# mjq11302010044/TPGSR

Measured on AMD Instinct MI355X. Metric: training img/s (16x64->32x128, bs=48/GPU), TPGSR-TSRN full train step, higher is better.
Workload: dtype bf16x2; 1 GPU; C3: TPGSR-TSRN = TSRN_TL (STN+mask) + CRNN teacher/student text prior, stu_iter 1, full train step (teacher fwd, student fwd+bwd, distill loss, prior dropout, SR fwd+bwd, ImageLoss(gradient), clip 0.25, Adam); tpg=crnn, batch_per_gpu=48, global_batch=48, parallelism=dp1, launch=recorded plans, plain launches: main + weight-gradient + teacher streams

## Files before the change

include/tpgsr_hip.h:

```cpp
#ifndef TPGSR_HIP_H
#define TPGSR_HIP_H

#ifdef __cplusplus
extern "C" {
#endif

#define TPGSR_ACT_NONE 0
#define TPGSR_ACT_RELU 1
#define TPGSR_ACT_MISH 2
#define TPGSR_ACT_TANH 3
#define TPGSR_ACT_PRELU 4

const char* tpgsr_last_error(void);
int tpgsr_version(void);
int tpgsr_sizeof(int which);

typedef struct {
  const float* in;
  const float* in2;
  const float* in_scale;
  const float* in_shift;
  const float* wt;
  const float* bias;
  float* out;
  float* bn_partial;
  int N, H, W, Cin;
// ... 137 lines not shown
  float* dwih0;
  float* dwih1;
  float* dbih0;
  float* dbih1;
  int Cin, U, G, blk0;
} tpgsr_compose_bwd_desc;
int tpgsr_compose_bwd_blocks(int Cin, int U, int G);
int tpgsr_compose_bwd_program(const tpgsr_compose_bwd_desc* descs_dev, int ndesc, int total_blocks, void* stream);
int tpgsr_pack_blocks(int kind, int Cout, int Cin, int KH, int KW, long long numel);
int tpgsr_pack_program(const tpgsr_pack_desc* descs_dev, int ndesc, int total_blocks, void* stream);
typedef struct tpgsr_split_desc {
  const float* src;
  void* dst;
  int K, N, ld, kp, blk0;
  int cin;
} tpgsr_split_desc;
int tpgsr_split_bf_blocks(int K, int N);
int tpgsr_split_bf_program(const tpgsr_split_desc* descs_dev, int ndesc, int total_blocks, void* stream);
int tpgsr_bicubic_resize(const float* in_nchw, int N, int Ctot, int C, int H, int W, int OH, int OW, float scale, float shift,
                         float* out_nhwc, void* stream);
int tpgsr_bicubic_upsample(const float* in_nchw, int N, int Ctot, int C, int H, int W, int scale, float* out_nchw, void* stream);
int tpgsr_aster_attention(const float* xproj, const float* sproj, const float* wv, const float* bv, const float* x, int N, int T, int A,
                          int D, float* alpha, float* context, void* stream);
int tpgsr_embed_concat(const int* ids, const float* emb, int V, int E, const float* ctx, int D, int N, float* out, void* stream);
int tpgsr_gru_cell(const float* gi, const float* gh, const float* h, int N, int Hd, float* hnew, void* stream);
int tpgsr_softmax_max(const float* logits, int N, int C, int* ids, float* score, int ld, int col, int* ids_next, void* stream);
int tpgsr_aster_attention_rows(const float* xproj, const float* sproj, const float* wv, const float* bv, const float* x, int R,
                               int rows_per_seq, int T, int A, int D, float* alpha, float* context, void* stream);
int tpgsr_beam_step(const float* logits, float* seq, int N, int B, int C, int eos, float* score_t, int* sym_t, int* pred_t, void* stream);
int tpgsr_gather_rows(const float* src, const int* idx, int R, int W, float* dst, void* stream);
// ... 247 lines not shown
```

tpgsr_amd/csrc/conv_loader.h:

```cpp
#pragma once
#include "common.h"

#define BM 64
#define BN 64
#define KC 32
#define ALD (BM + 1)

__device__ __forceinline__ int xcd_remap(int L, int total) {
  int q = total >> 3, r = total & 7;
  int xcd = L & 7, j = L >> 3;
  return (xcd < r ? xcd * (q + 1) : r * (q + 1) + (xcd - r) * q) + j;
}

struct PixelPos {
  int n, oh, ow;
  bool valid;
};

__device__ __forceinline__ PixelPos decode_pixel(const tpgsr_conv_args& a, int m, int M) {
  PixelPos p;
  p.valid = m < M;
  int mm = p.valid ? m : 0;
  int ohw = a.OH * a.OW;
  p.n = mm / ohw;
// ... 108 lines not shown
  s.dr = dk - dq * a.Cin;
  s.dqh = dq / a.KW;
  s.dqw = dq - s.dqh * a.KW;
  return s;
}
__device__ __forceinline__ void kpos_advance(const tpgsr_conv_args& a, KPos& k, const KStep& s) {
  k.c += s.dr;
  const bool cc = k.c >= a.Cin;
  k.c -= cc ? a.Cin : 0;
  k.kw += s.dqw + (cc ? 1 : 0);
  const bool cw = k.kw >= a.KW;
  k.kw -= cw ? a.KW : 0;
  k.kh += s.dqh + (cw ? 1 : 0);
}

template <int LD>
__device__ __forceinline__ ARaw load_a_raw(const tpgsr_conv_args& a, __amdgpu_buffer_rsrc_t rin, __amdgpu_buffer_rsrc_t rin2,
                                           const PixelPos& p, const KPos& kp) {
  ARaw r;
  const int kh = kp.kh, kw = kp.kw, c = kp.c;
  int ih = p.oh + kh - a.pad_h, iw = p.ow * stride_w(a) + kw - a.pad_w;
  r.ok = p.valid && kh < a.KH && c < a.Cin && (unsigned)ih < (unsigned)a.H && (unsigned)iw < (unsigned)a.W;
  int Wr = a.W;
  if (a.in_dil_w > 1) {
    r.ok = r.ok && (iw % a.in_dil_w) == 0;
    iw /= a.in_dil_w;
    Wr = real_w(a);
  }
  const unsigned pix = (unsigned)((p.n * a.H + ih) * Wr + iw);
  if ((LD & 16) && c >= a.cin_a) {
    r.v = buf_load4(rin2, r.ok ? (((unsigned)p.n * (unsigned)Wr + (unsigned)iw) * (unsigned)a.in_b_ld + (unsigned)(c - a.cin_a)) * 4u : OOB_OFF);
    r.v2 = make_float4(0.f, 0.f, 0.f, 0.f);
    r.raw = true;
    return r;
  }
  r.raw = false;
  if (!(LD & 8)) {
    r.v = buf_load4(rin, r.ok ? (pix * (unsigned)a.in_ld + (unsigned)(a.in_coff + c)) * 4u : OOB_OFF);
  } else {
    unsigned C4 = (unsigned)a.Cin >> 2, cs = (unsigned)c >> 2, W2 = 2u * (unsigned)a.W;
    unsigned b = r.ok ? ((((unsigned)p.n * 2u * a.H + 2u * ih) * W2 + 2u * iw) * C4 + cs) * 4u : OOB_OFF;
    r.v.x = buf_load1(rin, b);
    r.v.y = buf_load1(rin, r.ok ? b + C4 * 4u : OOB_OFF);
    r.v.z = buf_load1(rin, r.ok ? b + W2 * C4 * 4u : OOB_OFF);
    r.v.w = buf_load1(rin, r.ok ? b + (W2 * C4 + C4) * 4u : OOB_OFF);
  }
  if (LD & 4) r.v2 = buf_load4(rin2, r.ok ? (pix * (unsigned)a.in2_ld + (unsigned)c) * 4u : OOB_OFF);
  return r;
}

template <int LD>
__device__ __forceinline__ float4 finish_a(const tpgsr_conv_args& a, const ARaw& r, const float4& s, const float4& t,
                                           const float4& s2 = make_float4(1.f, 1.f, 1.f, 1.f)) {
// ... 35 lines not shown
```

tpgsr_amd/csrc/conv_mfma.hip:

```cpp
#include "common.h"
#include <mutex>

#ifndef TPGSR_FRAG_PRELOAD
#define TPGSR_FRAG_PRELOAD 0
#endif
#include <utility>
#include <vector>
#include "conv_loader.h"
#include "conv_launch.h"

template <int LD, int SPLIT>
__global__ __launch_bounds__(256 * SPLIT) void conv_fwd_kernel(tpgsr_conv_args a, int M, int K, int vecB) {
  constexpr bool VEC_A = LD >= 0;
  __shared__ float As_[SPLIT][KC][ALD];
  __shared__ float Bs_[SPLIT][KC][BN];
  const int grp = SPLIT > 1 ? (int)(threadIdx.x >> 8) : 0;
  float (*As)[ALD] = As_[grp];
  float (*Bs)[BN] = Bs_[grp];
  const int tid = threadIdx.x & 255;
  const int lane = tid & 63, wave = tid >> 6;
  const int wm = wave & 1, wn = wave >> 1;
  const int nbn = (a.Cout + BN - 1) / BN;
  const int tile = xcd_remap(blockIdx.x, gridDim.x);
  const int mblk = tile / nbn;
// ... 324 lines not shown
  long long M = (long long)a->N * a->OH * a->OW;
  int K = a->KH * a->KW * a->Cin;
  TPGSR_CHECK_ARG(M < (1ll << 31), "tpgsr_conv_fwd: M too large");
  hipStream_t st = (hipStream_t)stream;
  if (a->bnb_y) {
    TPGSR_CHECK_ARG(!a->out_ps && !a->bias && a->out_act == TPGSR_ACT_NONE,
                    "tpgsr_conv_fwd: bnb_y goes with a plain dense data-gradient store (no bias, no output activation, no pixel shuffle)");
    TPGSR_CHECK_ARG(a->bnb_act == TPGSR_ACT_NONE || a->bnb_act == TPGSR_ACT_RELU || a->bnb_act == TPGSR_ACT_MISH, "tpgsr_conv_fwd: bnb_act %d", a->bnb_act);
    TPGSR_CHECK_ARG((a->bnb_scale == nullptr) == (a->bnb_shift == nullptr), "tpgsr_conv_fwd: bnb_scale / bnb_shift must come together");
    if (a->bn_partial)
      TPGSR_CHECK_ARG(a->bnb_mean && a->bnb_rstd && (a->bnb_act == TPGSR_ACT_NONE || a->bnb_scale),
                      "tpgsr_conv_fwd: BatchNorm-backward sums need bnb_mean, bnb_rstd (and bnb_scale / bnb_shift under an activation)");
    else
      TPGSR_CHECK_ARG(a->bnb_store_dz, "tpgsr_conv_fwd: bnb_y without bn_partial and without bnb_store_dz does nothing");
  }
  const bool xbf = xbf_eligible(a);
  if (xbf) {
    TPGSR_CHECK_ARG(a->terms >= 1 && a->terms <= 3, "tpgsr_conv_fwd: terms must be 0, 1, 2 or 3");
    TPGSR_CHECK_ARG(a->kp >= K && (a->kp & 31) == 0 && ((uintptr_t)a->wt_bf & 15) == 0, "tpgsr_conv_fwd: bad split operand (kp %d, K %d)", a->kp, K);
    TPGSR_CHECK_ARG(a->wt_bf_cin == 0 || (a->wt_bf_cin == a->Cin && (a->Cin & 31) == 0),
                    "tpgsr_conv_fwd: weights were split in channel-block order for Cin %d, the convolution has Cin %d", a->wt_bf_cin, a->Cin);
  } else {
    TPGSR_CHECK_ARG(a->bn_row_tiles <= 1, "tpgsr_conv_fwd: bn_row_tiles %d needs the whole-CU halo kernel (split-bf16 path)", a->bn_row_tiles);
    TPGSR_CHECK_ARG(!a->bnb_y, "tpgsr_conv_fwd: the BatchNorm-backward epilogue (bnb_y) exists in the split-bf16 kernels only (terms > 0, wt_bf, Cin %% 4 == 0)");
  }
  const tpgsr_conv_route_t r = conv_fwd_route(a, M);
  if (xbf && a->sk_splits <= 1 && r.kernel != TPGSR_CONV_XBF_HALO3) {
    TPGSR_CHECK_ARG(!(r.ld & 32), "tpgsr_conv_fwd: a scaled residual operand (in2_scale) exists in the whole-CU halo kernel's loader only, which does not "
                    "take this launch (ask tpgsr_conv_in2_scale_ok first)");
    TPGSR_CHECK_ARG(a->bn_row_tiles <= 1, "tpgsr_conv_fwd: bn_row_tiles %d is the whole-CU halo kernel's, which does not take this launch "
                    "(ask tpgsr_conv_bn_row_tiles first)", a->bn_row_tiles);
  }
  dim3 grid(cdiv(M, BM) * cdiv(a->Cout, BN));
  switch (r.kernel) {
    case TPGSR_CONV_XBF_SPLITK:
    case TPGSR_CONV_XBF_TILE: return conv_fwd_xbf_launch(a, M, K, r, st);
// ... 741 lines not shown
```

tpgsr_amd/csrc/conv_xbf.hip:

```cpp
#include "conv_loader.h"
#include <type_traits>
#include <utility>
#include <vector>
#include <mutex>

#include "conv_xbf_common.h"

__device__ __forceinline__ int xa_off(int row, int slot) { return row * 64 + ((slot ^ ((row >> 2) & 3)) << 4); }

template <int LD, int T, int WMB, int WNB, int SK = 0>
__global__ __launch_bounds__(256, (WMB * WNB == 1 ? 3 : WMB * WNB == 2 ? 2 : 1)) void conv_fwd_xbf_kernel(tpgsr_conv_args a, int M, int K) {
  constexpr int BMT = 64 * WMB, BNT = 64 * WNB;
  constexpr int A_PLANE = BMT * 64;
  constexpr int BUF = T * A_PLANE;
  constexpr int NQ = BMT / 32;
  constexpr bool TWO = (T == 3) && (WMB * WNB <= 2);
  constexpr int EPI = (4 * 64 * WNB + 4 * 1024) * 4;
  __shared__ __attribute__((aligned(16))) unsigned char xsm[2 * BUF > EPI ? 2 * BUF : EPI];
  const int tid = threadIdx.x;
  const int lane = tid & 63, wave = tid >> 6;
  const int wm = wave & 1, wn = wave >> 1;
  const int nbn = (a.Cout + BNT - 1) / BNT;
  const int ntile = SK ? (int)gridDim.x / a.sk_splits : (int)gridDim.x;
  const int skz = SK ? (int)blockIdx.x / ntile : 0;
// ... 33 lines not shown
  ARaw qa[NQ];
  float4 qs = make_float4(1.f, 1.f, 1.f, 1.f), qt = make_float4(0.f, 0.f, 0.f, 0.f);
  const bool kperm = a.wt_bf_cin > 0;
  KPos kp_ = kperm ? KPos{0, 0, aq * 4} : kpos_init(a, aq);
  if (SK && c0 > 0) {
    if (kperm) {
      const int taps = a.KH * a.KW, cb = c0 / taps, tp = c0 - cb * taps;
      kp_ = KPos{tp / a.KW, tp - (tp / a.KW) * a.KW, cb * 32 + aq * 4};
    } else {
      kpos_advance(a, kp_, c0 * KC);
    }
  }
  const KStep kstep = kstep_init(a, KC);
  auto load_chunk = [&]() {
#pragma unroll
    for (int i = 0; i < NQ; ++i) qa[i] = load_a_raw<LD>(a, rs_in, rs_in2, px[i], kp_);
    if (LD & 1) {
      qs = *reinterpret_cast<const float4*>(a.in_scale + ((kp_.kh < a.KH && kp_.c < a.Cin) ? kp_.c : 0));
      qt = *reinterpret_cast<const float4*>(a.in_shift + ((kp_.kh < a.KH && kp_.c < a.Cin) ? kp_.c : 0));
    }
    if (kperm) {
      const bool cw = ++kp_.kw >= a.KW;
      kp_.kw = cw ? 0 : kp_.kw;
      kp_.kh += cw ? 1 : 0;
      const bool chh = kp_.kh >= a.KH;
      kp_.kh = chh ? 0 : kp_.kh;
      kp_.c += chh ? 32 : 0;
    } else {
      kpos_advance(a, kp_, kstep);
    }
  };
// ... 240 lines not shown
      }
    };
    constexpr bool DB = !(LD & 4);
    ARaw hr[DB ? 2 : 1][NE];
    float4 qs[2], qt[2];
    qs[0] = qs[1] = make_float4(1.f, 1.f, 1.f, 1.f);
    qt[0] = qt[1] = make_float4(0.f, 0.f, 0.f, 0.f);
    auto load_item = [&](auto set_tag, const int cc) __attribute__((always_inline)) {
      constexpr int S = decltype(set_tag)::value;
      const int c = cc * 32 + aq * 4;
#pragma unroll
      for (int i = 0; i < NE; ++i) {
        const bool ok = hpix[i] >= 0;
        hr[S][i].ok = ok;
        hr[S][i].raw = hpix[i] > -2;
        if (LD & 8) {
          const unsigned C4 = (unsigned)a.Cin >> 2, W2 = 2u * (unsigned)a.W;
          const unsigned b = ok ? ((2u * (unsigned)hpix[i] * W2 + 2u * (unsigned)hcol[i]) * C4 + ((unsigned)c >> 2)) * 4u : OOB_OFF;
          hr[S][i].v.x = buf_load1(rs_in, b);
          hr[S][i].v.y = buf_load1(rs_in, ok ? b + C4 * 4u : OOB_OFF);
          hr[S][i].v.z = buf_load1(rs_in, ok ? b + W2 * C4 * 4u : OOB_OFF);
          hr[S][i].v.w = buf_load1(rs_in, ok ? b + (W2 * C4 + C4) * 4u : OOB_OFF);
        } else {
          hr[S][i].v = buf_load4(rs_in, ok ? ((unsigned)hpix[i] * (unsigned)a.in_ld + (unsigned)(a.in_coff + c)) * 4u : OOB_OFF);
        }
        if (LD & 4) hr[S][i].v2 = buf_load4(rs_in2, ok ? ((unsigned)hpix[i] * (unsigned)a.in2_ld + (unsigned)c) * 4u : OOB_OFF);
      }
      if (LD & 1) {
        qs[S] = *reinterpret_cast<const float4*>(a.in_scale + c);
        qt[S] = *reinterpret_cast<const float4*>(a.in_shift + c);
      }
// ... 683 lines not shown
  const int lane = threadIdx.x & 63;
  const long long b = (long long)blockIdx.x * 4 + (threadIdx.x >> 6);
  if (b >= (long long)MB16 * NB32) return;
  const int mb = (int)(b / NB32), nb = (int)(b - (long long)mb * NB32);
  const int n = nb * 32 + (lane & 31), p0 = mb * 16 + (lane >> 5) * 8;
  __bf16 h[8][T];
#pragma unroll
  for (int j = 0; j < 8; ++j) {
    const int m = p0 + j;
    float v = 0.f;
    if (m < M && n < Cout) {
      if (!dy_ps) {
        v = dy[(size_t)m * dy_ld + dy_coff + n];
      } else {
        const int ohw = OH * OW, nn = m / ohw, rem = m - nn * ohw, oh = rem / OW, ow = rem - oh * OW;
        v = dy[((size_t)(nn * 2 * OH + 2 * oh + ((n >> 1) & 1)) * (2 * OW) + 2 * ow + (n & 1)) * (Cout >> 2) + (n >> 2)];
      }
    }
    split_bf<T>(v, h[j]);
  }
  const size_t plane = (size_t)MB16 * NB32 * 512;
#pragma unroll
  for (int t = 0; t < T; ++t) {
    bf16x8 v;
#pragma unroll
    for (int j = 0; j < 8; ++j) v[j] = h[j][t];
    *reinterpret_cast<bf16x8*>(out + t * plane + ((size_t)b * 64 + lane) * 8) = v;
  }
}

struct FastDiv {
// ... 234 lines not shown
          }
        }
      }
    };
    if (!(dbg & 1)) {
      step(I0{}, 0, t * 4 + 0);
      step(I1{}, 1, t * 4 + 1);
      step(I0{}, 2, t * 4 + 2);
      step(I1{}, 3, t * 4 + 3);
    }
  }

  const int n = n0 + wn * 32 + (lane & 31);
  float* dst = w.part + (size_t)z * K * a.Cout;
  if (n < a.Cout) {
#pragma unroll
    for (int i = 0; i < 3; ++i)
      if (i < ntap) {
#pragma unroll
        for (int r = 0; r < 16; ++r) {
          const int k = (tap0 + i) * a.Cin + cc * 32 + (r & 3) + 8 * (r >> 2) + 4 * (lane >> 5);
          dst[(size_t)k * a.Cout + n] = acc[i][r];
        }
      }
    if (want_db && lane < 32) w.dbpart[(size_t)z * a.Cout + n] = accdb[0];
  }
}

extern "C" int tpgsr_wgrad_halo_plan(const tpgsr_conv_args* a, int* zsplits, long long* dy_bf_bytes) {
  if (!a) return 0;
  int cus = 256, dev = 0;
  if (hipGetDevice(&dev) == hipSuccess) (void)hipDeviceGetAttribute(&cus, hipDeviceAttributeMultiprocessorCount, dev);
  if (cus < 1) cus = 256;
  return wgrad_halo_plan(a, cus, zsplits, dy_bf_bytes);
}

int conv_wgrad_halo_launch(const tpgsr_wgrad_args* w, long long M, const tpgsr_wgrad_route_t& r, hipStream_t st) {
  const tpgsr_conv_args* a = &w->c;
  const int T = a->terms, ld = r.ld, Lcap = r.lcap;
  const size_t lds = r.lds_bytes;
// ... 53 lines not shown
  __syncthreads();
  const tpgsr_split_desc d = descs[s_d];
  const int b = (int)blockIdx.x - d.blk0;
  const int nkb = d.kp / 64 + ((d.kp & 63) ? 1 : 0);
  const int kb = b % nkb, nbk = b / nkb;
  const int k0 = kb * 64, n0 = nbk * 64;
  {
    const int n = threadIdx.x & 63, kr = threadIdx.x >> 6;
#pragma unroll
    for (int i = 0; i < 16; ++i) {
      int k = k0 + kr * 16 + i;
      if (d.cin > 0 && k < d.K) {
        const int taps = d.K / d.cin, cc = k / (taps * 32), rem = k - cc * taps * 32;
        k = (rem >> 5) * d.cin + cc * 32 + (rem & 31);
      }
      tile[kr * 16 + i][n] = (k < d.K && n0 + n < d.N) ? d.src[(size_t)k * d.ld + n0 + n] : 0.f;
    }
  }
  __syncthreads();
  const int NB32 = (d.N + 31) >> 5, KB16 = d.kp >> 4;
  unsigned short* dst = reinterpret_cast<unsigned short*>(d.dst);
  const size_t plane = (size_t)NB32 * KB16 * 512;
  for (int i = 0; i < 2; ++i) {
    const int p = threadIdx.x + 256 * i;
    const int n = p & 63, kg = p >> 6;
    const int k = k0 + kg * 8, nn = n0 + n;
    if (k >= d.kp || nn >= NB32 * 32) continue;
    __bf16 h[8][3];
#pragma unroll
    for (int j = 0; j < 8; ++j) split_bf<3>(tile[kg * 8 + j][n], h[j]);
    const size_t off = ((((size_t)(nn >> 5) * KB16 + (k >> 4)) * 64) + ((k >> 3) & 1) * 32 + (nn & 31)) * 8;
// ... 60 lines not shown
```

tpgsr_amd/csrc/conv_xbf_common.h:

```cpp
#pragma once
#include "conv_loader.h"
#include "conv_launch.h"

typedef __bf16 bf16x8 __attribute__((ext_vector_type(8)));
typedef __bf16 bf16x4 __attribute__((ext_vector_type(4)));
typedef short s16x4 __attribute__((ext_vector_type(4)));
typedef __attribute__((address_space(3))) s16x4* lds_s16x4_ptr;

#define XW_ROW 192
#define XW_PLANE (32 * XW_ROW)

template <int T>
__device__ __forceinline__ void split_bf(float x, __bf16 (&h)[T]) {
  h[0] = (__bf16)x;
  if (T > 1) {
    float r = x - (float)h[0];
    h[1] = (__bf16)r;
    if (T > 2) h[2] = (__bf16)(r - (float)h[1]);
  }
}
template <int T>
__device__ __forceinline__ void split4(const float4& v, uint2 (&out)[T]) {
  __bf16 a[T], b[T], c[T], d[T];
  split_bf<T>(v.x, a);
// ... 22 lines not shown
    acc = __builtin_amdgcn_mfma_f32_32x32x16_bf16(a[1], b[0], acc, 0, 0, 0);
  }
  return __builtin_amdgcn_mfma_f32_32x32x16_bf16(a[0], b[0], acc, 0, 0, 0);
}

#ifndef XBF_NT_STORE
#define XBF_NT_STORE 0
#endif
__device__ __forceinline__ float xbf_bnb_elem(float raw, float y, float sc, float sh, float mu, float rs, int act, float& s, float& ss) {
  const float dz = act ? raw * act_grad(__builtin_fmaf(y, sc, sh), act) : raw;
  s += dz;
  ss = __builtin_fmaf(dz * (y - mu), rs, ss);
  return dz;
}

template <int WMB, int WNB>
__device__ __forceinline__ void xbf_store_tile(const tpgsr_conv_args& a, floatx16 (&acc)[WMB][WNB], int M, int m0, int n0, int wm,
                                               int wn, int lane, float* red) {
  constexpr int BNT = 64 * WNB;
  const int ohw = a.OH * a.OW;
#pragma unroll
  for (int j = 0; j < WNB; ++j) {
    const int cloc = wn * 32 * WNB + 32 * j + (lane & 31);
    const int n = n0 + cloc;
    const bool nvalid = n < a.Cout;
    const float bias = (a.bias && nvalid) ? a.bias[n] : 0.f;
    float s = 0.f, ss = 0.f;
    const bool bnb = a.bnb_y != nullptr;
    float b_mu = 0.f, b_rs = 0.f, b_sc = 1.f, b_sh = 0.f;
    if (bnb && nvalid) {
      if (a.bn_partial) {
        b_mu = a.bnb_mean[n];
        b_rs = a.bnb_rstd[n];
// ... 112 lines not shown
__device__ __forceinline__ void xbf_bn_flush(const tpgsr_conv_args& a, int M, int n0, int mblk, int tid, const float* red) {
  constexpr int BNT = 64 * WNB;
  for (int e = tid; e < BNT * WMB; e += 256) {
    const int blk = e / BNT, c = e - blk * BNT;
    const long long rb64 = (long long)mblk * WMB + blk;
    if (n0 + c < a.Cout && rb64 * 64 < M) {
      float* dst = a.bn_partial + (size_t)rb64 * 2 * a.Cout;
      float v0, v1;
      if (WMB == 1) {
        v0 = red[0 * BNT + c] + red[2 * BNT + c];
        v1 = red[1 * BNT + c] + red[3 * BNT + c];
      } else {
        v0 = red[(blk * 2 + 0) * BNT + c];
        v1 = red[(blk * 2 + 1) * BNT + c];
      }
      dst[n0 + c] = v0;
      dst[a.Cout + n0 + c] = v1;
    }
  }
}

template <int WMB, int WNB>
__device__ __forceinline__ void xbf_epilogue(const tpgsr_conv_args& a, floatx16 (&acc)[WMB][WNB], int M, int m0, int n0, int mblk,
                                             int wm, int wn, int lane, int tid, float* red, float* stage = nullptr) {
  xbf_store_tile_wide<WMB, WNB>(a, acc, M, m0, n0, wm, wn, lane, red, stage);
  if (a.bn_partial) {
    __syncthreads();
    xbf_bn_flush<WMB, WNB>(a, M, n0, mblk, tid, red);
  }
}
```

tpgsr_amd/engine.py:

```python
from __future__ import annotations

import contextlib
import ctypes as C
import math
import os
from typing import Dict, List, Optional

import torch

from . import kernels as K
from ._lib import PackDesc
from .kernels import ConvGeom, Plan, recording

F32 = torch.float32


class ParamArena:

    def __init__(self, module: torch.nn.Module):
        self.module = module
        self.flat: Optional[torch.Tensor] = None
        self.grad: Optional[torch.Tensor] = None
        self.offsets: Dict[str, int] = {}
        self.numel = 0
# ... 132 lines not shown

    def __call__(self, name, *shape, dtype=F32):
        t = self.t.get(name)
        if t is None:
            t = torch.empty(*shape, dtype=dtype, device=self.device)
            self.t[name] = t
        assert tuple(t.shape) == tuple(shape), (name, tuple(t.shape), shape)
        return t

    def nbytes(self):
        return sum(t.numel() * t.element_size() for t in self.t.values() if isinstance(t, torch.Tensor))


class ConvLayer:
    def __init__(self, eng, wname: str, bname: Optional[str], KH=1, KW=1, pad_h=0, pad_w=0, wscale=1.0, tail=False,
                 need_dgrad=True):
        self.eng, self.wname, self.bname, self.tail, self.wscale = eng, wname, bname, tail, wscale
        self.w = eng.P[wname]
        self.b = eng.P[bname] if bname else None
        dev = eng.device
        if tail:
            Co, Cc, KS, _ = self.w.shape
            self.Co, self.KS = Co, KS
            self.Cout, self.Cin, self.KH, self.KW, self.pad_h, self.pad_w = KS * Co, Cc, KS, 1, KS // 2, 0
        else:
            self.Cout, self.Cin = self.w.shape[0], self.w.shape[1]
            self.KH, self.KW, self.pad_h, self.pad_w = KH, KW, pad_h, pad_w
        Kd = self.KH * self.KW * self.Cin
        self.wt_f = torch.empty(Kd, self.Cout, dtype=F32, device=dev)
        self.wt_d = torch.empty(self.KH * self.KW * self.Cout, self.Cin, dtype=F32, device=dev) if need_dgrad else None
        if tail:
            eng.add_pack(self.w, self.wt_f, self.wt_d, Cout=self.Co, Cin=self.Cin, KH=self.KS, KW=self.KS, kind=1)
        else:
            eng.add_pack(self.w, self.wt_f, self.wt_d, Cout=self.Cout, Cin=self.Cin, KH=KH, KW=KW, kind=0,
                         f_ld=self.Cout, wscale=wscale)
        eng.register_operand(self.wt_f, self.wt_d, cins=(self.Cin, self.Cout))

    def geom(self, N, H, W) -> ConvGeom:
        return ConvGeom(N, H, W, self.Cin, self.Cout, self.KH, self.KW, self.pad_h, self.pad_w)

    def fwd(self, N, H, W, x, out, *, use_bias=True, **kw) -> ConvGeom:
        g = self.geom(N, H, W)
        a = K.make_conv_args(g, x, self.wt_f, out, bias=self.b if (use_bias and not self.tail) else None, **kw)
        K.conv_fwd(a)
        g.bn_row_tiles = max(1, a.bn_row_tiles)
        return g

    def dgrad(self, N, H, W, dy, dx, **kw):
        K.conv_fwd(K.make_conv_args(self.geom(N, H, W).dgrad(), dy, self.wt_d, dx, **kw))

    def wgrad(self, N, H, W, x, dy, *, loader: dict = None, dy_kw: dict = None):
# ... 289 lines not shown
                setattr(d, k, v.data_ptr())
            keep += list(t.values())
            d.Cin, d.U, d.G, d.blk0 = L.Cin, L.U, L.G, blk
            blk += lib.tpgsr_compose_bwd_blocks(L.Cin, L.U, L.G)
        table = torch.frombuffer(bytearray(bytes(arr)), dtype=torch.uint8).to(self.device)
        if K._REC is not None:
            K._REC.keep += keep
        with K.side():
            K.compose_bwd_program(table, len(items), blk)

    def add_pack(self, src, dst_f, dst_d, Cout=0, Cin=0, KH=1, KW=1, kind=0, f_ld=0, f_coff=0, wscale=1.0, src2=None, src3=None,
                 numel=None, d_ld=0, cin_ld=0):
        self._pack.append((src, dst_f, dst_d, Cout, Cin, KH, KW, kind, f_ld, f_coff, wscale, src2, src3, numel, d_ld, cin_ld,
                           getattr(self, "_pack_group", 0)))

    def register_operand(self, *tensors, cins=None):
        for i, t in enumerate(tensors):
            if t is not None:
                assert t.dim() == 2 and t.is_contiguous()
                self._operands.append(t)
                t._tpgsr_cin = K.block_order_cin(t.shape[0], cins[i] if cins else 0)
                t._tpgsr_group = getattr(self, "_pack_group", 0)

    def _finish_split_table(self):
        from ._lib import SplitDesc, load
        self._split_tabs = {}
        self._split_n = 0
        ops, seen = [], set()
        for t in self._operands:
            if t.data_ptr() not in seen:
                seen.add(t.data_ptr())
                ops.append(t)
        if K.POLICY == "f32" or not ops:
            return
        lib = load()
        self._split_keep = []
        for grp in sorted({getattr(t, "_tpgsr_group", 0) for t in ops}):
            sel = [t for t in ops if getattr(t, "_tpgsr_group", 0) == grp]
            arr = (SplitDesc * len(sel))()
            blk = 0
            for d, t in zip(arr, sel):
                Kd, N = t.shape
                kp = (Kd + 31) // 32 * 32
                twin = torch.zeros(3 * ((N + 31) // 32 * 32) * kp, dtype=torch.bfloat16, device=self.device)
                cin = getattr(t, "_tpgsr_cin", 0)
                K.register_bf_twin(t, twin, kp, cin)
                d.src, d.dst, d.K, d.N, d.ld, d.kp, d.blk0, d.cin = t.data_ptr(), twin.data_ptr(), Kd, N, N, kp, blk, cin
                blk += lib.tpgsr_split_bf_blocks(Kd, N)
                self._split_keep += [t, twin]
            self._split_tabs[grp] = (torch.frombuffer(bytearray(bytes(arr)), dtype=torch.uint8).to(self.device), len(sel), blk)
        self._split_n = len(ops)

    def _finish_pack_table(self):
        from ._lib import load
        lib = load()
        self._pack_tabs = {}
        self._pack_keep = []
        for grp in sorted({e[16] for e in self._pack}):
            sel = [e for e in self._pack if e[16] == grp]
            arr = (PackDesc * len(sel))()
            blk = 0
            for d, (src, dst_f, dst_d, Cout, Cin, KH, KW, kind, f_ld, f_coff, wscale, src2, src3, numel, d_ld, cin_ld, _g) in zip(arr, sel):
# ... 141 lines not shown
                gru1=g1, gru2=GruLayer(self, p + ".gru2", axis=0)))
        if self.tl:
            cfg = [(2, 1), (2, 1), (2, 1), (1, 0)]
            self.ig = [TConvStrip(self, f"infoGen.tconv{i + 1}.weight", sw, pw) for i, (sw, pw) in enumerate(cfg)]
            self.ig_bn = [BNLayer(self, f"infoGen.bn{i + 1}") for i in range(4)]
            self.Ct = self.ig[3].Cout
            self.emb_cls = self.ig[0].Cin
        k7 = f"block{self.srb + 2}"
        self.conv7 = ConvLayer(self, k7 + ".0.weight", k7 + ".0.bias", 3, 3, 1, 1)
        self.bn7 = BNLayer(self, k7 + ".1")
        k8 = f"block{self.srb + 3}"
        self.n_up = len([k for k in self.P if k.startswith(k8 + ".") and k.endswith(".conv.weight")])
        if self.n_up < 1:
            raise NotImplementedError("TSRN without an up-sampling block (scale_factor = 1) is not on the TPGSR hot path")
        assert self.scale == 2 ** self.n_up
        self.ups = [ConvLayer(self, f"{k8}.{k}.conv.weight", f"{k8}.{k}.conv.bias", 3, 3, 1, 1) for k in range(self.n_up)]
        self.tail = ConvLayer(self, f"{k8}.{self.n_up}.weight", None, tail=True)
        self.tail_bias = self.P[f"{k8}.{self.n_up}.bias"]
        if self.stn:
            self.stn_convs, self.stn_bns = [], []
            for i in range(6):
                cp = f"stn_head.stn_convnet.{2 * i}"
                self.stn_convs.append(ConvLayer(self, cp + ".0.weight", cp + ".0.bias", 3, 3, 1, 1, need_dgrad=(i > 0)))
                self.stn_bns.append(BNLayer(self, cp + ".1"))
            w1 = self.P["stn_head.stn_fc1.0.weight"]
            self.fc1 = _FC1AsConv(self, "stn_head.stn_fc1.0.weight", "stn_head.stn_fc1.0.bias", w1.shape[0], w1.shape[1] // 2)
            self.bnf = BNLayer(self, "stn_head.stn_fc1.1")
            self.fc2 = ConvLayer(self, "stn_head.stn_fc2.weight", "stn_head.stn_fc2.bias", wscale=0.1)
            self.tps_inv = self.B["tps.inverse_kernel"]
            self.tps_repr = self.B["tps.target_coordinate_repr"]
            self.NC = self.B["tps.target_control_points"].shape[0]
# ... 418 lines not shown
```

tpgsr_amd/functional.py:

```python
from __future__ import annotations

from contextlib import contextmanager, nullcontext
from typing import Optional, Sequence, Tuple

import torch

from . import kernels as K
from .kernels import ConvGeom

F32 = torch.float32


def _chk(*ts):
    for t in ts:
        if t is None:
            continue
        if not (t.is_cuda or K.DRYRUN):
            raise RuntimeError("tpgsr_amd.functional runs on the GPU only (no CPU / stock-PyTorch fallback)")
        if t.dtype != F32:
            raise TypeError(f"tpgsr_amd.functional expects fp32 tensors, got {t.dtype}")


def _new(like, *shape):
    return torch.empty(*shape, dtype=F32, device=like.device)
# ... 92 lines not shown
    def backward(ctx, g):
        N, C, H, W = g.shape
        out = _new(g, N, H, W, C)
        K.nchw_to_nhwc(_c(g), N, C, H, W, out)
        return out


def to_nhwc(x):
    return _ToNHWC.apply(x)


def to_nchw(x):
    return _ToNCHW.apply(x)


def _pack(w, transposed, wscale):
    if transposed:
        Cin, Cout, KH, KW = w.shape
    else:
        Cout, Cin, KH, KW = w.shape
    wt_f = torch.empty(KH * KW * Cin, Cout, dtype=F32, device=w.device)
    wt_d = torch.empty(KH * KW * Cout, Cin, dtype=F32, device=w.device)
    K.pack_conv_weight(_c(w), Cout, Cin, KH, KW, wt_f, wt_d, transposed=transposed, wscale=wscale)
    if K.CONV_TERMS:
        K.make_bf_twin(wt_f, Cin)
        K.make_bf_twin(wt_d, Cout)
    return wt_f, wt_d, Cout, Cin, KH, KW


class _Conv2d(torch.autograd.Function):

    @staticmethod
    def forward(ctx, x, w, b, pad_h, pad_w, out_ps, transposed, wscale):
        _chk(x, w, b)
        x = _c(x)
        N, H, W, Cx = x.shape
        wt_f, wt_d, Cout, Cin, KH, KW = _pack(w, transposed, wscale)
        if Cx != Cin:
            raise ValueError(f"conv2d: input has {Cx} channels, weight expects {Cin}")
        g = ConvGeom(N, H, W, Cin, Cout, KH, KW, pad_h, pad_w)
        if g.OH <= 0 or g.OW <= 0:
            raise ValueError("conv2d: empty output")
        out = _new(x, N, 2 * g.OH, 2 * g.OW, Cout // 4) if out_ps else _new(x, N, g.OH, g.OW, Cout)
        K.conv_fwd(K.make_conv_args(g, x, wt_f, out, bias=b, out_ps=out_ps))
        ctx.save_for_backward(x, w, wt_d, b)
        ctx.cfg = (g, out_ps, transposed, wscale)
        return out

    @staticmethod
    def backward(ctx, dy):
        x, w, wt_d, b = ctx.saved_tensors
        g, out_ps, transposed, wscale = ctx.cfg
# ... 81 lines not shown
    KH, KW = w.shape[2], w.shape[3]
    xd = x if (sh == 1 and sw == 1) else _Dilate.apply(x, sh, sw)
    return _Conv2d.apply(xd, w, None, KH - 1 - ph, KW - 1 - pw, False, True, 1.0)


class _TConvK4S2SubPixel(torch.autograd.Function):

    @staticmethod
    def forward(ctx, x, w):
        _chk(x, w)
        x = _c(x)
        N, H, W, Cx = x.shape
        Cin, Cout = w.shape[0], w.shape[1]
        w3 = _new(x, 4 * Cout, Cin, 3, 3)
        K.tconv4s2_expand(_c(w), Cin, Cout, w3)
        wt_f, wt_d, *_ = _pack(w3, False, 1.0)
        g = ConvGeom(N, H, W, Cin, 4 * Cout, 3, 3, 1, 1)
        out = _new(x, N, 2 * H, 2 * W, Cout)
        K.conv_fwd(K.make_conv_args(g, x, wt_f, out, out_ps=True))
        ctx.save_for_backward(x, w, wt_d)
        ctx.g = g
        return out

    @staticmethod
    def backward(ctx, dy):
        x, w, wt_d = ctx.saved_tensors
        g = ctx.g
        Cin, Cout = w.shape[0], w.shape[1]
        dy = _c(dy)
        dx = dw = None
        if ctx.needs_input_grad[0]:
# ... 840 lines not shown
```

tpgsr_amd/kernels.py:

```python
from __future__ import annotations

import ctypes as C
import os
from dataclasses import dataclass
from typing import Optional

import torch

from . import _lib
from ._lib import ConvArgs, GruWgradArgs, WgradArgs, act_code, check


DRYRUN = os.environ.get("TPGSR_PLAN_DRYRUN") == "1"


_TERMS = {"f32": 0, "x3": 3, "bf16": 1, "x2": 2, "x3b2": 3}
_X2_TPG_FWD = int(os.environ.get("TPGSR_X2_TPG_FWD", "3"))
POLICY = os.environ.get("TPGSR_CONV_PREC", "x3")
if POLICY not in _TERMS:
    raise ValueError(f"TPGSR_CONV_PREC={POLICY!r}: expected one of {sorted(_TERMS)}")
CONV_TERMS = _TERMS[POLICY]


_POLICY_EXPLICIT = "TPGSR_CONV_PREC" in os.environ
# ... 47 lines not shown
class conv_terms:

    def __init__(self, terms):
        self.terms = terms

    def __enter__(self):
        global CONV_TERMS
        self.prev, CONV_TERMS = CONV_TERMS, self.terms

    def __exit__(self, *exc):
        global CONV_TERMS
        CONV_TERMS = self.prev
        return False


def register_bf_twin(wt: torch.Tensor, twin: torch.Tensor, kp: int, cin: int = 0):
    wt._tpgsr_twin = (twin, kp, cin)


def block_order_cin(Kd: int, cin: int) -> int:
    return cin if (cin and cin % 32 == 0 and Kd % cin == 0 and Kd // cin > 1) else 0


class _DummyStream:
    cuda_stream = None
    device = torch.device("cpu")

    def wait_stream(self, other):
        pass

    def __enter__(self):
        return self
# ... 460 lines not shown
    a.out_act = act_code(out_act)
    a.out_ps = int(bool(out_ps))
    a.in_b = _p(in_b)
    a.cin_a = cin_a if in_b is not None else 0
    a.in_b_ld = (g.Cin - cin_a) if in_b_ld is None else in_b_ld
    a.in_dil_w = in_dil_w
    a.wt_ld, a.wt_coff = wt_ld, wt_coff
    a.stride_w = stride_w
    a.terms = 0
    if CONV_TERMS and g.Cin % 4 == 0:
        if wt is None or isinstance(wt, (int, DynPtr)):
            a.terms = CONV_TERMS
        else:
            tw = getattr(wt, "_tpgsr_twin", None)
            if tw is not None:
                a.terms, a.kp, a.wt_bf, a.wt_bf_cin = CONV_TERMS, tw[1], tw[0].data_ptr(), tw[2]
                a._dev = tw[0].device
                assert tw[2] in (0, g.Cin), f"operand split for Cin {tw[2]}, used by a convolution over {g.Cin} channels"
                if _REC is not None:
                    _REC.keep.append(tw[0])
    if bnb is not None:
        if not (a.terms and a.wt_bf and wt_coff % 32 == 0):
            raise RuntimeError("BatchNorm-backward statistics ride on the split-bf16 convolution kernels only (check bnb_fusable first)")
        a.bn_partial = _p(bnb.get("partial"))
        a.bnb_y, a.bnb_mean, a.bnb_rstd = _p(bnb["y"]), _p(bnb.get("mean")), _p(bnb.get("rstd"))
        a.bnb_scale, a.bnb_shift, a.bnb_act = _p(bnb.get("scale")), _p(bnb.get("shift")), act_code(bnb["act"])
        a.bnb_store_dz = int(bool(bnb.get("store_dz", False)))
    if (bn_coarse or (bnb is not None and bnb.get("coarse"))) and a.bn_partial and BN_COARSE_ROWS and CONV_TERMS:
        if _lib.load().tpgsr_conv_bn_row_tiles(C.byref(a)) == 3:
            a.bn_row_tiles = 3
    if bnb is not None:
        bnb["row_tiles"] = max(1, a.bn_row_tiles)
    return a
# ... 602 lines not shown
    _launch("tpgsr_col2im3x3_c1", _p(dcol), N, H, W, _p(din))


def pad_channels(src, M, Cs, Cd, dst):
    _launch("tpgsr_pad_channels", _p(src), M, Cs, Cd, _p(dst))


def semantic_loss_fwd(p, q, n, partial, nblk):
    _launch("tpgsr_semantic_loss_fwd", _p(p), _p(q), n, _p(partial), nblk)


def semantic_loss_bwd(p, q, dloss, n, dp):
    _launch("tpgsr_semantic_loss_bwd", _p(p), _p(q), _p(dloss), n, _p(dp))


def make_bf_twin(wt: torch.Tensor, cin: int = 0):
    lib = _lib.load()
    Kd, N = wt.shape
    cin = block_order_cin(Kd, cin)
    kp = (Kd + 31) // 32 * 32
    twin = torch.zeros(3 * ((N + 31) // 32 * 32) * kp, dtype=torch.bfloat16, device=wt.device)
    d = (_lib.SplitDesc * 1)()
    d[0].src, d[0].dst, d[0].K, d[0].N, d[0].ld, d[0].kp, d[0].blk0, d[0].cin = wt.data_ptr(), twin.data_ptr(), Kd, N, N, kp, 0, cin
    table = torch.frombuffer(bytearray(bytes(d)), dtype=torch.uint8).to(wt.device)
    split_bf_program(table, 1, lib.tpgsr_split_bf_blocks(Kd, N))
    register_bf_twin(wt, twin, kp, cin)
    return twin, kp


def split_bf_program(descs_dev, ndesc, total_blocks):
    _launch("tpgsr_split_bf_program", _p(descs_dev), ndesc, total_blocks)


def copy_strided(src, src_ld, src_coff, dst, dst_ld, dst_coff, M, C_, accumulate=False):
    _launch("tpgsr_copy_strided", _p(src), src_ld, src_coff, _p(dst), dst_ld, dst_coff, M, C_, int(accumulate))


def resize_nearest_fwd(inp, N, H, W, C_, s, out):
    _launch("tpgsr_resize_nearest_fwd", _p(inp), N, H, W, C_, s, _p(out))


# ... 170 lines not shown
```

Baseline: 8798 img/s.

## Reorder split-bf16 weight planes into pixel-shuffle order for upsample convs

The split-bf16 weight twins of the TSRN upsampling convolutions are permuted into pixel-shuffle channel order, flagged by a tag bit in the wt_bf pointer. The forward epilogue can then write each output pixel's four shuffled channels as one contiguous float4 after a DPP quad transpose, and the in_ps loaders read four consecutive channels with a single vector load instead of four scattered scalar loads. The weight-gradient writeback, bias and BN statistics indices are mapped back to the original column order. This adds index remapping, pointer tagging and new validation checks, and a wrong permutation anywhere would silently corrupt results.

```diff
diff --git a/include/tpgsr_hip.h b/include/tpgsr_hip.h
--- a/include/tpgsr_hip.h
+++ b/include/tpgsr_hip.h
@@ -10,6 +10,7 @@
 #define TPGSR_ACT_MISH 2
 #define TPGSR_ACT_TANH 3
 #define TPGSR_ACT_PRELU 4
+#define TPGSR_WT_BF_PS 1
 
 const char* tpgsr_last_error(void);
 int tpgsr_version(void);
@@ -177,6 +178,8 @@
   void* dst;
   int K, N, ld, kp, blk0;
   int cin;
+  int ps;
+  int reserved;
 } tpgsr_split_desc;
 int tpgsr_split_bf_blocks(int K, int N);
 int tpgsr_split_bf_program(const tpgsr_split_desc* descs_dev, int ndesc, int total_blocks, void* stream);
diff --git a/tpgsr_amd/csrc/conv_loader.h b/tpgsr_amd/csrc/conv_loader.h
--- a/tpgsr_amd/csrc/conv_loader.h
+++ b/tpgsr_amd/csrc/conv_loader.h
@@ -146,7 +146,16 @@
   k.kh += s.dqh + (cw ? 1 : 0);
 }
 
-template <int LD>
+__host__ __device__ __forceinline__ int ps_orig(int np, int C) {
+  const int q = np / C;
+  return (np - q * C) * 4 + q;
+}
+__device__ __forceinline__ unsigned ps_index(unsigned np, unsigned C, unsigned n, unsigned h, unsigned w, unsigned H, unsigned W) {
+  const unsigned q = (np >= C ? 1u : 0u) + (np >= 2u * C ? 1u : 0u) + (np >= 3u * C ? 1u : 0u);
+  return (((n * 2u * H + 2u * h + (q >> 1)) * (2u * W)) + 2u * w + (q & 1u)) * C + (np - q * C);
+}
+
+template <int LD, bool PSQ = false>
 __device__ __forceinline__ ARaw load_a_raw(const tpgsr_conv_args& a, __amdgpu_buffer_rsrc_t rin, __amdgpu_buffer_rsrc_t rin2,
                                            const PixelPos& p, const KPos& kp) {
   ARaw r;
@@ -169,6 +178,8 @@
   r.raw = false;
   if (!(LD & 8)) {
     r.v = buf_load4(rin, r.ok ? (pix * (unsigned)a.in_ld + (unsigned)(a.in_coff + c)) * 4u : OOB_OFF);
+  } else if (PSQ && a.reserved2) {
+    r.v = buf_load4(rin, r.ok ? ps_index((unsigned)c, (unsigned)a.Cin >> 2, (unsigned)p.n, (unsigned)ih, (unsigned)iw, (unsigned)a.H, (unsigned)a.W) * 4u : OOB_OFF);
   } else {
     unsigned C4 = (unsigned)a.Cin >> 2, cs = (unsigned)c >> 2, W2 = 2u * (unsigned)a.W;
     unsigned b = r.ok ? ((((unsigned)p.n * 2u * a.H + 2u * ih) * W2 + 2u * iw) * C4 + cs) * 4u : OOB_OFF;
diff --git a/tpgsr_amd/csrc/conv_mfma.hip b/tpgsr_amd/csrc/conv_mfma.hip
--- a/tpgsr_amd/csrc/conv_mfma.hip
+++ b/tpgsr_amd/csrc/conv_mfma.hip
@@ -362,12 +362,25 @@
     else
       TPGSR_CHECK_ARG(a->bnb_store_dz, "tpgsr_conv_fwd: bnb_y without bn_partial and without bnb_store_dz does nothing");
   }
+  const bool ps_planes = ((uintptr_t)a->wt_bf & TPGSR_WT_BF_PS) != 0;
+  tpgsr_conv_args unmarked;
+  if (ps_planes) {
+    unmarked = *a;
+    unmarked.wt_bf = (const void*)((uintptr_t)a->wt_bf & ~(uintptr_t)TPGSR_WT_BF_PS);
+    unmarked.reserved2 = 1;
+    a = &unmarked;
+  }
   const bool xbf = xbf_eligible(a);
   if (xbf) {
     TPGSR_CHECK_ARG(a->terms >= 1 && a->terms <= 3, "tpgsr_conv_fwd: terms must be 0, 1, 2 or 3");
     TPGSR_CHECK_ARG(a->kp >= K && (a->kp & 31) == 0 && ((uintptr_t)a->wt_bf & 15) == 0, "tpgsr_conv_fwd: bad split operand (kp %d, K %d)", a->kp, K);
     TPGSR_CHECK_ARG(a->wt_bf_cin == 0 || (a->wt_bf_cin == a->Cin && (a->Cin & 31) == 0),
                     "tpgsr_conv_fwd: weights were split in channel-block order for Cin %d, the convolution has Cin %d", a->wt_bf_cin, a->Cin);
+    TPGSR_CHECK_ARG(!(a->out_ps && a->in_ps), "tpgsr_conv_fwd: out_ps and in_ps together have no split-bf16 kernel");
+    TPGSR_CHECK_ARG(!ps_planes || a->out_ps || a->in_ps,
+                    "tpgsr_conv_fwd: planes in pixel-shuffle order (TPGSR_WT_BF_PS) handed to a launch that is neither out_ps nor in_ps");
+    if (a->in_ps && ps_planes) TPGSR_CHECK_ARG((a->Cin & 15) == 0, "tpgsr_conv_fwd: in_ps over planes in pixel-shuffle order needs Cin %% 16 == 0 (a quad = four channels of one pixel)");
+    if (a->out_ps && ps_planes) TPGSR_CHECK_ARG(a->wt_coff == 0 && (a->wt_ld == 0 || a->wt_ld == a->Cout), "tpgsr_conv_fwd: out_ps over planes in pixel-shuffle order takes no weight column window");
   } else {
     TPGSR_CHECK_ARG(a->bn_row_tiles <= 1, "tpgsr_conv_fwd: bn_row_tiles %d needs the whole-CU halo kernel (split-bf16 path)", a->bn_row_tiles);
     TPGSR_CHECK_ARG(!a->bnb_y, "tpgsr_conv_fwd: the BatchNorm-backward epilogue (bnb_y) exists in the split-bf16 kernels only (terms > 0, wt_bf, Cin %% 4 == 0)");
diff --git a/tpgsr_amd/csrc/conv_xbf.hip b/tpgsr_amd/csrc/conv_xbf.hip
--- a/tpgsr_amd/csrc/conv_xbf.hip
+++ b/tpgsr_amd/csrc/conv_xbf.hip
@@ -71,7 +71,7 @@
   const KStep kstep = kstep_init(a, KC);
   auto load_chunk = [&]() {
 #pragma unroll
-    for (int i = 0; i < NQ; ++i) qa[i] = load_a_raw<LD>(a, rs_in, rs_in2, px[i], kp_);
+    for (int i = 0; i < NQ; ++i) qa[i] = load_a_raw<LD, true>(a, rs_in, rs_in2, px[i], kp_);
     if (LD & 1) {
       qs = *reinterpret_cast<const float4*>(a.in_scale + ((kp_.kh < a.KH && kp_.c < a.Cin) ? kp_.c : 0));
       qt = *reinterpret_cast<const float4*>(a.in_shift + ((kp_.kh < a.KH && kp_.c < a.Cin) ? kp_.c : 0));
@@ -342,7 +342,9 @@
         const bool ok = hpix[i] >= 0;
         hr[S][i].ok = ok;
         hr[S][i].raw = hpix[i] > -2;
-        if (LD & 8) {
+        if ((LD & 8) && a.reserved2) {
+          hr[S][i].v = buf_load4(rs_in, ok ? ps_index((unsigned)c, (unsigned)a.Cin >> 2, 0u, (unsigned)hpix[i], (unsigned)hcol[i], (unsigned)a.H, (unsigned)a.W) * 4u : OOB_OFF);
+        } else if (LD & 8) {
           const unsigned C4 = (unsigned)a.Cin >> 2, W2 = 2u * (unsigned)a.W;
           const unsigned b = ok ? ((2u * (unsigned)hpix[i] * W2 + 2u * (unsigned)hcol[i]) * C4 + ((unsigned)c >> 2)) * 4u : OOB_OFF;
           hr[S][i].v.x = buf_load1(rs_in, b);
@@ -1056,7 +1058,7 @@
         v = dy[(size_t)m * dy_ld + dy_coff + n];
       } else {
         const int ohw = OH * OW, nn = m / ohw, rem = m - nn * ohw, oh = rem / OW, ow = rem - oh * OW;
-        v = dy[((size_t)(nn * 2 * OH + 2 * oh + ((n >> 1) & 1)) * (2 * OW) + 2 * ow + (n & 1)) * (Cout >> 2) + (n >> 2)];
+        v = dy[ps_index((unsigned)n, (unsigned)Cout >> 2, (unsigned)nn, (unsigned)oh, (unsigned)ow, (unsigned)OH, (unsigned)OW)];
       }
     }
     split_bf<T>(v, h[j]);
@@ -1321,16 +1323,17 @@
   const int n = n0 + wn * 32 + (lane & 31);
   float* dst = w.part + (size_t)z * K * a.Cout;
   if (n < a.Cout) {
+    const int col = w.dy_ps ? ps_orig(n, a.Cout >> 2) : n;
 #pragma unroll
     for (int i = 0; i < 3; ++i)
       if (i < ntap) {
 #pragma unroll
         for (int r = 0; r < 16; ++r) {
           const int k = (tap0 + i) * a.Cin + cc * 32 + (r & 3) + 8 * (r >> 2) + 4 * (lane >> 5);
-          dst[(size_t)k * a.Cout + n] = acc[i][r];
+          dst[(size_t)k * a.Cout + col] = acc[i][r];
         }
       }
-    if (want_db && lane < 32) w.dbpart[(size_t)z * a.Cout + n] = accdb[0];
+    if (want_db && lane < 32) w.dbpart[(size_t)z * a.Cout + col] = accdb[0];
   }
 }
 
@@ -1414,7 +1417,12 @@
         const int taps = d.K / d.cin, cc = k / (taps * 32), rem = k - cc * taps * 32;
         k = (rem >> 5) * d.cin + cc * 32 + (rem & 31);
       }
-      tile[kr * 16 + i][n] = (k < d.K && n0 + n < d.N) ? d.src[(size_t)k * d.ld + n0 + n] : 0.f;
+      if (d.ps < 0 && k < d.K) {
+        const int cin = -4 * d.ps, tap = k / cin;
+        k = tap * cin + ps_orig(k - tap * cin, -d.ps);
+      }
+      const int col = (d.ps > 0 && n0 + n < d.N) ? ps_orig(n0 + n, d.ps) : n0 + n;
+      tile[kr * 16 + i][n] = (k < d.K && n0 + n < d.N) ? d.src[(size_t)k * d.ld + col] : 0.f;
     }
   }
   __syncthreads();
diff --git a/tpgsr_amd/csrc/conv_xbf_common.h b/tpgsr_amd/csrc/conv_xbf_common.h
--- a/tpgsr_amd/csrc/conv_xbf_common.h
+++ b/tpgsr_amd/csrc/conv_xbf_common.h
@@ -60,9 +60,88 @@
   return dz;
 }
 
+__device__ __forceinline__ float xbf_quad_xor(float v, int which) {
+  const int x = __float_as_int(v);
+  return __int_as_float(which == 1 ? __builtin_amdgcn_update_dpp(x, x, 0xB1, 0xF, 0xF, false)
+                                   : __builtin_amdgcn_update_dpp(x, x, 0x4E, 0xF, 0xF, false));
+}
+__device__ __forceinline__ void xbf_quad_transpose(float (&v)[4], int lane) {
+  const bool o1 = lane & 1, o2 = lane & 2;
+#pragma unroll
+  for (int t = 0; t < 4; t += 2) {
+    const float got = xbf_quad_xor(o1 ? v[t] : v[t + 1], 1);
+    if (o1) v[t] = got; else v[t + 1] = got;
+  }
+#pragma unroll
+  for (int t = 0; t < 2; ++t) {
+    const float got = xbf_quad_xor(o2 ? v[t] : v[t + 2], 2);
+    if (o2) v[t] = got; else v[t + 2] = got;
+  }
+}
+
+template <int WMB, int WNB>
+__device__ __forceinline__ void xbf_store_tile_ps(const tpgsr_conv_args& a, floatx16 (&acc)[WMB][WNB], int M, int m0, int n0, int wm,
+                                                  int wn, int lane, float* red) {
+  constexpr int BNT = 64 * WNB;
+  const int ohw = a.OH * a.OW, C = a.Cout >> 2;
+  const bool wide = (C & 3) == 0 && ((uintptr_t)a.out & 15) == 0;
+  auto index = [&](int m, int np) __attribute__((always_inline)) {
+    const int nn = m / ohw, rem = m - nn * ohw, oh = rem / a.OW, ow = rem - oh * a.OW;
+    const int q = np / C;
+    return ((size_t)(nn * 2 * a.OH + 2 * oh + (q >> 1)) * (2 * a.OW) + 2 * ow + (q & 1)) * C + (np - q * C);
+  };
+#pragma unroll
+  for (int j = 0; j < WNB; ++j) {
+    const int cloc = wn * 32 * WNB + 32 * j + (lane & 31);
+    const int n = n0 + cloc;
+    const bool nvalid = n < a.Cout;
+    const float bias = (a.bias && nvalid) ? a.bias[ps_orig(n, C)] : 0.f;
+    const int nq = n0 + wn * 32 * WNB + 32 * j + (lane & 28);
+    float s = 0.f, ss = 0.f;
+#pragma unroll
+    for (int i = 0; i < WMB; ++i) {
+      const int mrow0 = m0 + wm * 32 * WMB + 32 * i + 4 * (lane >> 5);
+#pragma unroll
+      for (int g = 0; g < 4; ++g) {
+        float v[4];
+#pragma unroll
+        for (int t = 0; t < 4; ++t) {
+          const float raw = acc[i][j][4 * g + t];
+          if (mrow0 + 8 * g + t < M && nvalid) {
+            s += raw;
+            ss = __builtin_fmaf(raw, raw, ss);
+          }
+          v[t] = apply_act(raw + bias, a.out_act);
+        }
+        if (wide) {
+          xbf_quad_transpose(v, lane);
+          const int m = mrow0 + 8 * g + (lane & 3);
+          if (m < M && nq < a.Cout) *reinterpret_cast<float4*>(a.out + index(m, nq)) = make_float4(v[0], v[1], v[2], v[3]);
+        } else {
+#pragma unroll
+          for (int t = 0; t < 4; ++t)
+            if (mrow0 + 8 * g + t < M && nvalid) a.out[index(mrow0 + 8 * g + t, n)] = v[t];
+        }
+      }
+    }
+    if (a.bn_partial) {
+      s += __shfl_xor(s, 32);
+      ss += __shfl_xor(ss, 32);
+      if (lane < 32) {
+        red[(wm * 2 + 0) * BNT + cloc] = s;
+        red[(wm * 2 + 1) * BNT + cloc] = ss;
+      }
+    }
+  }
+}
+
 template <int WMB, int WNB>
 __device__ __forceinline__ void xbf_store_tile(const tpgsr_conv_args& a, floatx16 (&acc)[WMB][WNB], int M, int m0, int n0, int wm,
                                                int wn, int lane, float* red) {
+  if (a.out_ps && a.reserved2) {
+    xbf_store_tile_ps<WMB, WNB>(a, acc, M, m0, n0, wm, wn, lane, red);
+    return;
+  }
   constexpr int BNT = 64 * WNB;
   const int ohw = a.OH * a.OW;
 #pragma unroll
@@ -205,8 +284,9 @@
         v0 = red[(blk * 2 + 0) * BNT + c];
         v1 = red[(blk * 2 + 1) * BNT + c];
       }
-      dst[n0 + c] = v0;
-      dst[a.Cout + n0 + c] = v1;
+      const int col = (a.out_ps && a.reserved2) ? ps_orig(n0 + c, a.Cout >> 2) : n0 + c;
+      dst[col] = v0;
+      dst[a.Cout + col] = v1;
     }
   }
 }
diff --git a/tpgsr_amd/engine.py b/tpgsr_amd/engine.py
--- a/tpgsr_amd/engine.py
+++ b/tpgsr_amd/engine.py
@@ -170,8 +170,8 @@
 
 class ConvLayer:
     def __init__(self, eng, wname: str, bname: Optional[str], KH=1, KW=1, pad_h=0, pad_w=0, wscale=1.0, tail=False,
-                 need_dgrad=True):
-        self.eng, self.wname, self.bname, self.tail, self.wscale = eng, wname, bname, tail, wscale
+                 need_dgrad=True, ps=False):
+        self.eng, self.wname, self.bname, self.tail, self.wscale, self.ps = eng, wname, bname, tail, wscale, bool(ps)
         self.w = eng.P[wname]
         self.b = eng.P[bname] if bname else None
         dev = eng.device
@@ -190,7 +190,7 @@
         else:
             eng.add_pack(self.w, self.wt_f, self.wt_d, Cout=self.Cout, Cin=self.Cin, KH=KH, KW=KW, kind=0,
                          f_ld=self.Cout, wscale=wscale)
-        eng.register_operand(self.wt_f, self.wt_d, cins=(self.Cin, self.Cout))
+        eng.register_operand(self.wt_f, self.wt_d, cins=(self.Cin, self.Cout), pss=(self.Cout // 4, -(self.Cout // 4) if self.Cout % 16 == 0 else 0) if ps else None)
 
     def geom(self, N, H, W) -> ConvGeom:
         return ConvGeom(N, H, W, self.Cin, self.Cout, self.KH, self.KW, self.pad_h, self.pad_w)
@@ -510,13 +510,14 @@
         self._pack.append((src, dst_f, dst_d, Cout, Cin, KH, KW, kind, f_ld, f_coff, wscale, src2, src3, numel, d_ld, cin_ld,
                            getattr(self, "_pack_group", 0)))
 
-    def register_operand(self, *tensors, cins=None):
+    def register_operand(self, *tensors, cins=None, pss=None):
         for i, t in enumerate(tensors):
             if t is not None:
                 assert t.dim() == 2 and t.is_contiguous()
                 self._operands.append(t)
                 t._tpgsr_cin = K.block_order_cin(t.shape[0], cins[i] if cins else 0)
                 t._tpgsr_group = getattr(self, "_pack_group", 0)
+                t._tpgsr_ps = pss[i] if pss else 0
 
     def _finish_split_table(self):
         from ._lib import SplitDesc, load
@@ -539,9 +540,9 @@
                 Kd, N = t.shape
                 kp = (Kd + 31) // 32 * 32
                 twin = torch.zeros(3 * ((N + 31) // 32 * 32) * kp, dtype=torch.bfloat16, device=self.device)
-                cin = getattr(t, "_tpgsr_cin", 0)
-                K.register_bf_twin(t, twin, kp, cin)
-                d.src, d.dst, d.K, d.N, d.ld, d.kp, d.blk0, d.cin = t.data_ptr(), twin.data_ptr(), Kd, N, N, kp, blk, cin
+                cin, ps = getattr(t, "_tpgsr_cin", 0), getattr(t, "_tpgsr_ps", 0)
+                K.register_bf_twin(t, twin, kp, cin, ps)
+                d.src, d.dst, d.K, d.N, d.ld, d.kp, d.blk0, d.cin, d.ps = t.data_ptr(), twin.data_ptr(), Kd, N, N, kp, blk, cin, ps
                 blk += lib.tpgsr_split_bf_blocks(Kd, N)
                 self._split_keep += [t, twin]
             self._split_tabs[grp] = (torch.frombuffer(bytearray(bytes(arr)), dtype=torch.uint8).to(self.device), len(sel), blk)
@@ -713,7 +714,7 @@
         if self.n_up < 1:
             raise NotImplementedError("TSRN without an up-sampling block (scale_factor = 1) is not on the TPGSR hot path")
         assert self.scale == 2 ** self.n_up
-        self.ups = [ConvLayer(self, f"{k8}.{k}.conv.weight", f"{k8}.{k}.conv.bias", 3, 3, 1, 1) for k in range(self.n_up)]
+        self.ups = [ConvLayer(self, f"{k8}.{k}.conv.weight", f"{k8}.{k}.conv.bias", 3, 3, 1, 1, ps=True) for k in range(self.n_up)]
         self.tail = ConvLayer(self, f"{k8}.{self.n_up}.weight", None, tail=True)
         self.tail_bias = self.P[f"{k8}.{self.n_up}.bias"]
         if self.stn:
diff --git a/tpgsr_amd/functional.py b/tpgsr_amd/functional.py
--- a/tpgsr_amd/functional.py
+++ b/tpgsr_amd/functional.py
@@ -130,7 +130,7 @@
     return _ToNCHW.apply(x)
 
 
-def _pack(w, transposed, wscale):
+def _pack(w, transposed, wscale, ps=False):
     if transposed:
         Cin, Cout, KH, KW = w.shape
     else:
@@ -139,8 +139,8 @@
     wt_d = torch.empty(KH * KW * Cout, Cin, dtype=F32, device=w.device)
     K.pack_conv_weight(_c(w), Cout, Cin, KH, KW, wt_f, wt_d, transposed=transposed, wscale=wscale)
     if K.CONV_TERMS:
-        K.make_bf_twin(wt_f, Cin)
-        K.make_bf_twin(wt_d, Cout)
+        K.make_bf_twin(wt_f, Cin, ps=Cout // 4 if ps else 0)
+        K.make_bf_twin(wt_d, Cout, ps=-(Cout // 4) if (ps and Cout % 16 == 0) else 0)
     return wt_f, wt_d, Cout, Cin, KH, KW
 
 
@@ -151,7 +151,7 @@
         _chk(x, w, b)
         x = _c(x)
         N, H, W, Cx = x.shape
-        wt_f, wt_d, Cout, Cin, KH, KW = _pack(w, transposed, wscale)
+        wt_f, wt_d, Cout, Cin, KH, KW = _pack(w, transposed, wscale, ps=out_ps)
         if Cx != Cin:
             raise ValueError(f"conv2d: input has {Cx} channels, weight expects {Cin}")
         g = ConvGeom(N, H, W, Cin, Cout, KH, KW, pad_h, pad_w)
@@ -263,7 +263,7 @@
         Cin, Cout = w.shape[0], w.shape[1]
         w3 = _new(x, 4 * Cout, Cin, 3, 3)
         K.tconv4s2_expand(_c(w), Cin, Cout, w3)
-        wt_f, wt_d, *_ = _pack(w3, False, 1.0)
+        wt_f, wt_d, *_ = _pack(w3, False, 1.0, ps=True)
         g = ConvGeom(N, H, W, Cin, 4 * Cout, 3, 3, 1, 1)
         out = _new(x, N, 2 * H, 2 * W, Cout)
         K.conv_fwd(K.make_conv_args(g, x, wt_f, out, out_ps=True))
diff --git a/tpgsr_amd/kernels.py b/tpgsr_amd/kernels.py
--- a/tpgsr_amd/kernels.py
+++ b/tpgsr_amd/kernels.py
@@ -85,8 +85,21 @@
         return False
 
 
-def register_bf_twin(wt: torch.Tensor, twin: torch.Tensor, kp: int, cin: int = 0):
-    wt._tpgsr_twin = (twin, kp, cin)
+WT_BF_PS = _lib.ABI.defines["TPGSR_WT_BF_PS"]
+
+
+def register_bf_twin(wt: torch.Tensor, twin: torch.Tensor, kp: int, cin: int = 0, ps: int = 0):
+    check_split_ps(wt, ps)
+    wt._tpgsr_twin = (twin, kp, cin, ps)
+
+
+def check_split_ps(wt: torch.Tensor, ps: int):
+    if ps and not (wt.shape[1] == 4 * ps if ps > 0 else wt.shape[0] % (-4 * ps) == 0):
+        raise ValueError(f"pixel-shuffle order {ps} does not fit an operand of shape {tuple(wt.shape)}")
+
+
+def ps_order_of(g: "ConvGeom", out_ps=False, in_ps=False) -> int:
+    return g.Cout // 4 if out_ps else -(g.Cin // 4) if (in_ps and g.Cin % 16 == 0) else 0
 
 
 def block_order_cin(Kd: int, cin: int) -> int:
@@ -577,9 +590,14 @@
         else:
             tw = getattr(wt, "_tpgsr_twin", None)
             if tw is not None:
-                a.terms, a.kp, a.wt_bf, a.wt_bf_cin = CONV_TERMS, tw[1], tw[0].data_ptr(), tw[2]
+                a.terms, a.kp, a.wt_bf_cin = CONV_TERMS, tw[1], tw[2]
                 a._dev = tw[0].device
                 assert tw[2] in (0, g.Cin), f"operand split for Cin {tw[2]}, used by a convolution over {g.Cin} channels"
+                ps = tw[3] if len(tw) > 3 else 0
+                if ps and ps != ps_order_of(g, out_ps, in_ps):
+                    raise ValueError(f"operand split in pixel-shuffle order {ps}, used by a launch that needs {ps_order_of(g, out_ps, in_ps)} "
+                                     f"(out_ps {bool(out_ps)}, in_ps {bool(in_ps)}, Cin {g.Cin}, Cout {g.Cout})")
+                a.wt_bf = tw[0].data_ptr() | (WT_BF_PS if ps else 0)
                 if _REC is not None:
                     _REC.keep.append(tw[0])
     if bnb is not None:
@@ -1212,17 +1230,19 @@
     _launch("tpgsr_semantic_loss_bwd", _p(p), _p(q), _p(dloss), n, _p(dp))
 
 
-def make_bf_twin(wt: torch.Tensor, cin: int = 0):
+def make_bf_twin(wt: torch.Tensor, cin: int = 0, ps: int = 0):
     lib = _lib.load()
+    check_split_ps(wt, ps)
     Kd, N = wt.shape
     cin = block_order_cin(Kd, cin)
     kp = (Kd + 31) // 32 * 32
     twin = torch.zeros(3 * ((N + 31) // 32 * 32) * kp, dtype=torch.bfloat16, device=wt.device)
     d = (_lib.SplitDesc * 1)()
     d[0].src, d[0].dst, d[0].K, d[0].N, d[0].ld, d[0].kp, d[0].blk0, d[0].cin = wt.data_ptr(), twin.data_ptr(), Kd, N, N, kp, 0, cin
+    d[0].ps = ps
     table = torch.frombuffer(bytearray(bytes(d)), dtype=torch.uint8).to(wt.device)
     split_bf_program(table, 1, lib.tpgsr_split_bf_blocks(Kd, N))
-    register_bf_twin(wt, twin, kp, cin)
+    register_bf_twin(wt, twin, kp, cin, ps)
     return twin, kp
 
 
```

Result: no change. 8775 img/s (-0.3%).
